# fabrizio-m/TyPLONK

Measured on AMD Instinct MI355X. Metric: msm_g1_adds_per_s, higher is better.
Workload: dtype u32; 1 GPU; 2^20-term BLS12-381 G1 MSM (KZG commit of a 2^20-row polynomial), SRS [s^i]G with s=2, 1048579 points; window_bits=20, windows=13, parallelism=single GPU, fixed_base_tables=c=20, 13 tables per rank

## Files before the change

### typlonk_amd/build.py

```python
from __future__ import annotations

import os
import shutil
import subprocess

ROOT = os.path.dirname(os.path.dirname(os.path.abspath(__file__)))
CSRC = os.path.join(ROOT, "typlonk_amd", "csrc")
LIB = os.path.join(ROOT, "typlonk_amd", "libtyplonk_hip.so")


def _stale(out: str, srcs: list[str]) -> bool:
    if not os.path.exists(out):
        return True
    t = os.path.getmtime(out)
    return any(os.path.getmtime(s) > t for s in srcs if os.path.exists(s))


def _run(cmd: list[str]) -> None:
    print("+", " ".join(cmd), flush=True)
    subprocess.run(cmd, check=True)


def hipcc_path() -> str:
    p = shutil.which("hipcc") or "/opt/rocm/bin/hipcc"
    if not os.path.exists(p):
        raise RuntimeError("hipcc not found: the HIP library cannot be built (there is no CPU fallback)")
    return p


HIP_UNITS = ["ctx.hip", "ntt_host.hip", "msm_host.hip", "comm.hip", "prover.hip", "ntt_kernels.hip", "msm_sort.hip", "msm_accum.hip", "msm_reduce.hip", "srs_gen.hip", "quotient.hip", "plonk_ops.hip", "poly_eval.hip", "verify.hip", "prove_batch.hip", "point_codec.hip", "witness_check.hip", "perm_pairs.hip", "witness_solve.hip"]
UNIT_FLAGS: dict[str, list[str]] = {}


def build_hip(force: bool = False) -> str:
    from concurrent.futures import ThreadPoolExecutor

    hdrs = [os.path.join(CSRC, f) for f in os.listdir(CSRC) if f.endswith(".hpp")]
    hdrs.append(os.path.join(ROOT, "include", "typlonk.h"))
    objdir = os.path.join(CSRC, "_obj")
    os.makedirs(objdir, exist_ok=True)
    hipcc = hipcc_path()
    jobs, objs = [], []
    for u in HIP_UNITS:
        src = os.path.join(CSRC, u)
        obj = os.path.join(objdir, u.replace(".hip", ".o"))
        objs.append(obj)
        if force or _stale(obj, [src] + hdrs):
            jobs.append([hipcc, "--offload-arch=gfx950", "-O3", "-std=c++17", "-fPIC", *UNIT_FLAGS.get(u, []), "-c", src, "-o", obj])
    if jobs:
        with ThreadPoolExecutor(max_workers=min(6, len(jobs))) as ex:
            list(ex.map(_run, jobs))
    if jobs or not os.path.exists(LIB):
        _run([hipcc, "--offload-arch=gfx950", "-shared", "-fPIC", *objs, "-o", LIB])
    return LIB


def build_hip_variant(name: str, unit_flags: dict[str, list[str]]) -> str:
    from concurrent.futures import ThreadPoolExecutor

    out_dir = os.path.join(ROOT, "tools", "_ab", name)
    os.makedirs(out_dir, exist_ok=True)
    hipcc = hipcc_path()
    base_obj = os.path.join(CSRC, "_obj")
    jobs, objs = [], []
    for u in HIP_UNITS:
        if u in unit_flags:
            obj = os.path.join(out_dir, u.replace(".hip", ".o"))
            jobs.append([hipcc, "--offload-arch=gfx950", "-O3", "-std=c++17", "-fPIC", *UNIT_FLAGS.get(u, []), *unit_flags[u], "-c",
                         os.path.join(CSRC, u), "-o", obj])
        else:
            obj = os.path.join(base_obj, u.replace(".hip", ".o"))
        objs.append(obj)
    build_hip()
    with ThreadPoolExecutor(max_workers=min(6, max(1, len(jobs)))) as ex:
        list(ex.map(_run, jobs))
    lib = os.path.join(out_dir, "libtyplonk_hip.so")
    _run([hipcc, "--offload-arch=gfx950", "-shared", "-fPIC", *objs, "-o", lib])
    return lib


def build_hip_test_hooks(force: bool = False) -> str:
    out_dir = os.path.join(ROOT, "tests", "cpp", "hooks")
    os.makedirs(out_dir, exist_ok=True)
    lib = os.path.join(out_dir, "libtyplonk_hip.so")
    hipcc = hipcc_path()
    build_hip()
    hdrs = [os.path.join(CSRC, f) for f in os.listdir(CSRC) if f.endswith(".hpp")] + [os.path.join(ROOT, "include", "typlonk.h")]
    src = os.path.join(CSRC, "comm.hip")
    obj = os.path.join(out_dir, "comm.o")
    base_obj = os.path.join(CSRC, "_obj")
    objs = [obj if u == "comm.hip" else os.path.join(base_obj, u.replace(".hip", ".o")) for u in HIP_UNITS]
    if force or _stale(obj, [src] + hdrs + [LIB]):
        _run([hipcc, "--offload-arch=gfx950", "-O3", "-std=c++17", "-fPIC", "-DTYPLONK_TEST_HOOKS", "-c", src, "-o", obj])
    if force or _stale(lib, objs):
        _run([hipcc, "--offload-arch=gfx950", "-shared", "-fPIC", *objs, "-o", lib])
    return lib


def build_host_shim(force: bool = False) -> str:
    src = os.path.join(ROOT, "tests", "cpp", "ff_host_shim.cpp")
    out = os.path.join(ROOT, "tests", "cpp", "libff_host_shim.so")
    deps = [src, os.path.join(CSRC, "ff.hpp"), os.path.join(CSRC, "g1.hpp"), os.path.join(CSRC, "fq30.hpp"), os.path.join(CSRC, "g1_host64.hpp"),
            os.path.join(CSRC, "fr30.hpp"), os.path.join(CSRC, "fr_inv.hpp"), os.path.join(CSRC, "transcript.hpp"), os.path.join(CSRC, "lin_commit.hpp")]
    if force or _stale(out, deps):
        _run(["g++", "-O2", "-std=c++17", "-shared", "-fPIC", src, "-o", out])
    return out


def build_device_arith(force: bool = False) -> str:
    src = os.path.join(ROOT, "tests", "cpp", "device_arith.hip")
    out = os.path.join(ROOT, "tests", "cpp", "libdevice_arith.so")
    hdrs = [os.path.join(CSRC, f) for f in os.listdir(CSRC) if f.endswith(".hpp")]
    if force or _stale(out, [src] + hdrs):
        _run([hipcc_path(), "--offload-arch=gfx950", "-O3", "-std=c++17", "-fPIC", "-shared", src, "-o", out])
    return out


def build_device_reduce(force: bool = False) -> str:
    src = os.path.join(CSRC, "harness", "device_reduce.hip")
    out = os.path.join(ROOT, "tests", "cpp", "libdevice_reduce.so")
    deps = [os.path.join(CSRC, f) for f in os.listdir(CSRC) if f.endswith(".hpp")] + [os.path.join(CSRC, "msm_reduce.hip")]
    if force or _stale(out, [src] + deps):
        _run([hipcc_path(), "--offload-arch=gfx950", "-O3", "-std=c++17", "-fPIC", "-shared", src, "-o", out])
    return out


def build_fq30_pair_host(force: bool = False) -> str:
    src = os.path.join(ROOT, "tests", "cpp", "fq30_pair_host.cpp")
    out = os.path.join(ROOT, "tests", "cpp", "libfq30_pair_host.so")
    deps = [src, os.path.join(ROOT, "tests", "cpp", "fq30_pair_harness.hpp"), os.path.join(CSRC, "ff.hpp"), os.path.join(CSRC, "fq30.hpp")]
    if force or _stale(out, deps):
        _run(["g++", "-O2", "-std=c++17", "-shared", "-fPIC", src, "-o", out])
    return out


def build_sigma_cell_host(force: bool = False) -> str:
    src = os.path.join(ROOT, "tests", "cpp", "sigma_cell_host.cpp")
    out = os.path.join(ROOT, "tests", "cpp", "libsigma_cell_host.so")
    deps = [src, os.path.join(CSRC, "ff.hpp"), os.path.join(CSRC, "sigma_cell.hpp")]
    if force or _stale(out, deps):
        _run(["g++", "-O2", "-std=c++17", "-shared", "-fPIC", src, "-o", out])
    return out


# ... 1 lines not shown
    src = os.path.join(ROOT, "tests", "cpp", "perm_pairs_host.cpp")
    out = os.path.join(ROOT, "tests", "cpp", "perm_pairs_host")
    deps = [src, os.path.join(CSRC, "ff.hpp"), os.path.join(CSRC, "perm_pairs.hpp")]
    if force or _stale(out, deps):
        _run(["g++", "-O2", "-std=c++17", "-pthread", src, "-o", out])
    return out


def build_msm_plan_host(force: bool = False) -> str:
    src = os.path.join(ROOT, "tests", "cpp", "msm_plan_host.cpp")
    out = os.path.join(ROOT, "tests", "cpp", "msm_plan_host")
    deps = [src, os.path.join(CSRC, "ff.hpp"), os.path.join(CSRC, "msm_plan.hpp")]
    if force or _stale(out, deps):
        _run(["g++", "-O2", "-std=c++17", src, "-o", out])
    return out


def build_ntt_plan_host(force: bool = False) -> str:
    src = os.path.join(ROOT, "tests", "cpp", "ntt_plan_host.cpp")
    out = os.path.join(ROOT, "tests", "cpp", "ntt_plan_host")
    deps = [src, os.path.join(CSRC, "ff.hpp"), os.path.join(CSRC, "fr30.hpp"), os.path.join(CSRC, "ntt_args.hpp"), os.path.join(CSRC, "ntt_plan.hpp")]
    if force or _stale(out, deps):
        _run(["g++", "-O2", "-std=c++17", src, "-o", out])
    return out


def build_prove_plan_host(force: bool = False, sanitize: bool = False) -> str:
    src = os.path.join(ROOT, "tests", "cpp", "prove_plan_host.cpp")
    out = os.path.join(ROOT, "tests", "cpp", "prove_plan_host_san" if sanitize else "prove_plan_host")
    deps = [src] + [os.path.join(CSRC, h) for h in ("ff.hpp", "fr30.hpp", "ntt_args.hpp", "ntt_plan.hpp", "prove_plan.hpp")]
    if force or _stale(out, deps):
        extra = ["-O1", "-g", "-fsanitize=address,undefined", "-fno-sanitize-recover=all"] if sanitize else ["-O2"]
        _run(["g++", *extra, "-std=c++17", src, "-o", out])
    return out


def build_solve_plan_host(force: bool = False, sanitize: bool = False) -> str:
    src = os.path.join(ROOT, "tests", "cpp", "solve_plan_host.cpp")
    out = os.path.join(ROOT, "tests", "cpp", "solve_plan_host_san" if sanitize else "solve_plan_host")
    deps = [src, os.path.join(CSRC, "solve_plan.hpp")]
    if force or _stale(out, deps):
        extra = ["-O1", "-g", "-fsanitize=address,undefined", "-fno-sanitize-recover=all"] if sanitize else ["-O2"]
        _run(["g++", *extra, "-std=c++17", src, "-o", out])
    return out


def build_madd_acc_host(force: bool = False, sanitize: bool = False) -> str:
    src = os.path.join(ROOT, "tests", "cpp", "madd_acc_host.cpp")
    out = os.path.join(ROOT, "tests", "cpp", "madd_acc_host_san" if sanitize else "madd_acc_host")
    deps = [src, os.path.join(CSRC, "ff.hpp"), os.path.join(CSRC, "fq30.hpp"), os.path.join(CSRC, "g1.hpp")]
    if force or _stale(out, deps):
        extra = ["-O1", "-g", "-fsanitize=address,undefined", "-fno-sanitize-recover=all"] if sanitize else ["-O2"]
        _run(["g++", *extra, "-std=c++17", src, "-o", out])
    return out


def build_device_pair(force: bool = False) -> str:
    src = os.path.join(ROOT, "tests", "cpp", "device_pair.hip")
    out = os.path.join(ROOT, "tests", "cpp", "libdevice_pair.so")
    hdrs = [os.path.join(CSRC, f) for f in os.listdir(CSRC) if f.endswith(".hpp")]
    hdrs.append(os.path.join(ROOT, "tests", "cpp", "fq30_pair_harness.hpp"))
    if force or _stale(out, [src] + hdrs):
        _run([hipcc_path(), "--offload-arch=gfx950", "-O3", "-std=c++17", "-fPIC", "-shared", src, "-o", out])
    return out


def build_host_tests(force: bool = False) -> list[str]:
    outs = []
    hdr = [os.path.join(ROOT, "typlonk_amd", "host", "typlonk_host.hpp"), os.path.join(ROOT, "typlonk_amd", "host", "pairing_host.hpp"),
           os.path.join(ROOT, "tests", "cpp", "circuit_host.hpp"),
           os.path.join(CSRC, "ff.hpp"), os.path.join(CSRC, "fq30.hpp"), os.path.join(CSRC, "g1_host64.hpp"),
           os.path.join(CSRC, "transcript.hpp"), LIB]
    for name in ("test_poly_host", "test_kzg_host", "test_plonk_host", "test_pairing_host", "test_circuit_tables_host", "test_circuit_host",
                 "test_comm_host", "test_comm_ranks_host", "test_compact_ranks_host", "test_verify_host", "test_prove_batch_host", "test_compact_host",
                 "test_prove_batch_compact_host", "test_wire_host", "test_witness_check_host", "test_circuit_compile_host",
                 "test_circuit_pairs_host", "test_witness_solve_host"):
        src = os.path.join(ROOT, "tests", "cpp", name + ".cpp")
        out = os.path.join(ROOT, "tests", "cpp", name)
        if force or _stale(out, [src] + hdr):
            _run(["g++", "-O2", "-std=c++17", src, "-o", out, "-L", os.path.join(ROOT, "typlonk_amd"), "-ltyplonk_hip",
                  "-Wl,-rpath," + os.path.join(ROOT, "typlonk_amd"), "-Wl,-rpath,$ORIGIN/../../typlonk_amd"])
        outs.append(out)
    return outs


def build_fake_rccl(force: bool = False) -> str:
    src = os.path.join(ROOT, "tests", "cpp", "fake_rccl.cpp")
    out = os.path.join(ROOT, "tests", "cpp", "libfake_rccl.so")
    if force or _stale(out, [src]):
        _run([hipcc_path(), "-O2", "-std=c++17", "-shared", "-fPIC", "-x", "hip", "--offload-arch=gfx950", src, "-o", out, "-lrt"])
    return out


def build_all(force: bool = False) -> None:
    build_hip(force)
    build_hip_test_hooks(force)
    build_host_shim(force)
    build_device_arith(force)
    build_device_reduce(force)
    build_fq30_pair_host(force)
    build_sigma_cell_host(force)
    build_perm_pairs_host(force)
    if os.path.exists(os.path.join(ROOT, "tests", "cpp", "msm_plan_host.cpp")):
        build_msm_plan_host(force)
    if os.path.exists(os.path.join(ROOT, "tests", "cpp", "ntt_plan_host.cpp")):
        build_ntt_plan_host(force)
    if os.path.exists(os.path.join(ROOT, "tests", "cpp", "prove_plan_host.cpp")):
        build_prove_plan_host(force)
        build_prove_plan_host(force, sanitize=True)
    if os.path.exists(os.path.join(ROOT, "tests", "cpp", "madd_acc_host.cpp")):
        build_madd_acc_host(force)
        build_madd_acc_host(force, sanitize=True)
    if os.path.exists(os.path.join(ROOT, "tests", "cpp", "solve_plan_host.cpp")):
        build_solve_plan_host(force)
        build_solve_plan_host(force, sanitize=True)
    build_device_pair(force)
    build_host_tests(force)
    build_fake_rccl(force)


if __name__ == "__main__":
    import sys

    if len(sys.argv) >= 3 and sys.argv[1] == "variant":
        flags: dict[str, list[str]] = {}
        for spec in sys.argv[3:]:
            unit, _, fl = spec.partition(":")
            flags[unit] = [f for f in fl.split(",") if f]
        print(build_hip_variant(sys.argv[2], flags))
    else:
        build_all()
```

### typlonk_amd/csrc/launch.hpp

```cpp
#pragma once
#include <hip/hip_runtime.h>
#include <stdint.h>
#include "ff.hpp"
#include "msm_plan.hpp"
#include "ntt_args.hpp"

namespace ty {

constexpr int PT_WORDS = 32;
constexpr int MSM_HEAVY_GRID = 1024;

struct QuotientArgs {
    const Fr* wires[3];
    const Fr* z;
    const Fr* sel[5];
    const Fr* sigma[3];
    const Fr* pi;
    const Fr* l0;
    const Fr* w_lo;
    const Fr* bx_hi;
    Fr* out;
    uint64_t n4;
    uint32_t w_h;
    uint32_t k0_is_one;
// ... 15 lines not shown
    uint64_t n;
    uint32_t w_h;
    Fr beta, gamma;
    Fr kbeta[3];
};
void launch_gp_terms(const GrandProductArgs& a, hipStream_t s);
void launch_product_scan(const Fr* in, uint64_t n, int reverse, Fr* block_scratch, Fr* out, hipStream_t s);
void launch_fr_inv(const Fr* in, Fr* out, hipStream_t s);
void launch_gp_finish(const Fr* nprefix, const Fr* dsuffix, const Fr* inv_total , uint64_t n, Fr* z, hipStream_t s);

void launch_open(const Fr* c, uint64_t m, const Fr& z, Fr* q, Fr* blocks, Fr* y, hipStream_t s);
struct LincombArgs {
    const Fr* poly[12];
    Fr scalar[12];
    Fr constant;
    Fr* out;
    uint64_t n;
    uint32_t terms;
};
void launch_lincomb(const LincombArgs& a, hipStream_t s);
void launch_open_multi(const Fr* const* polys, Fr* const* quotients, Fr* const* ys, const uint8_t* zsel, uint32_t count,
                       uint64_t m, const Fr& z0, const Fr& z1, Fr* blocks, hipStream_t s);

bool ntt_big_tiles_available();
void launch_ntt_pass(const NttPassArgs& a, unsigned blocks, unsigned threads, size_t lds_bytes, hipStream_t s);
void launch_ntt_pass30(const NttPassArgs& a, unsigned blocks, unsigned threads, size_t lds_bytes, hipStream_t s);
void launch_ntt_full_table(const Fr* lo, const Fr* hi, uint32_t h, uint64_t S, uint64_t n, Fr* out, hipStream_t s);

void launch_convert_points(uint32_t* pts, const uint8_t* inf, uint64_t n, hipStream_t s);
void launch_msm_digits(const Fr* scalars, uint64_t m, uint32_t c, uint32_t W, uint32_t top_v, uint32_t* keys,
                       uint32_t* counts, hipStream_t s);
void launch_scan(const uint32_t* counts, uint64_t n, uint32_t* block_sums, uint32_t* offsets, uint32_t* cursor,
                 hipStream_t s);
struct MsmSortPtrs {
    uint32_t *blk_hist, *blk_base, *scan_scratch, *blk_cnt, *seg_start, *entries, *counts, *offsets, *sorted, *hist514, *heavy, *tasks,
        *order;
};
void launch_msm_segsort(const Fr* scalars, uint64_t m, const MsmShape& sh, const MsmSortPtrs& p, uint32_t cap, int staged_mode,
                        hipStream_t s);
size_t srs_tables_scratch_bytes(uint64_t len, uint32_t T);
void launch_srs_tables(uint32_t* pts, uint32_t* zbuf, uint64_t len, uint32_t c, uint32_t T, hipStream_t s);
void launch_bucket_order(const uint32_t* counts, const uint32_t* offsets, uint32_t n, uint32_t cap, uint32_t* hist514,
                         uint32_t* order, uint32_t* heavy, uint32_t* tasks, hipStream_t s);
void launch_msm_heavy(const uint32_t* points, const uint32_t* sorted, const uint32_t* hist516, uint32_t* heavy,
                      const uint32_t* tasks, uint32_t* partial, uint32_t* buckets, hipStream_t s);
void launch_msm_scatter(const uint32_t* keys, uint64_t m, uint64_t total, uint32_t* cursor, uint32_t* sorted,
                        hipStream_t s);
void launch_msm_accum(const uint32_t* points, const uint32_t* offsets, const uint32_t* sorted, const uint32_t* order,
                      uint32_t nbuckets, uint32_t cap, bool init, uint32_t lanes, uint32_t split, uint32_t* buckets,
                      hipStream_t s);

void launch_msm_rc_reduce(const uint32_t* buckets, const RcShape& sh, uint32_t* pb, uint32_t* pa, uint32_t* sums,
                          uint32_t* bitsum, uint32_t* out, hipStream_t s);
void launch_msm_rc2_reduce(const uint32_t* buckets, const RcShape& sh, uint32_t* prow, uint32_t* pcol, uint32_t* out,
                           hipStream_t s);
void launch_msm_rc_combine(const uint32_t* planes, const RcShape& sh, uint32_t* set_sums, hipStream_t s);
void launch_fq_inv_selftest(uint64_t seed, uint32_t threads, uint32_t per_thread, uint32_t* out, hipStream_t st);
size_t srs_comb_bytes();
void launch_srs_comb(uint32_t* comb, hipStream_t st);
void launch_srs_generate(const Fr& s, uint64_t start, uint64_t n, const uint32_t* comb, uint32_t* pts, hipStream_t st);

}
```

### typlonk_amd/csrc/msm_reduce.hip

```cpp
#include "launch.hpp"
#include "msm_common.hpp"

namespace ty {

__global__ __launch_bounds__(64) void msm_rc_partial_kernel(const uint32_t* __restrict__ buckets, RcShape sh,
                                                            uint32_t nrow, uint32_t nrow_pad, uint32_t ncol,
                                                            uint32_t* pb, uint32_t* pa) {
    const uint32_t t = blockIdx.x * 64 + threadIdx.x;
    if (t < nrow_pad) {
        if (t >= nrow) return;
        const uint64_t base = (uint64_t)t << sh.llc;
        G1Xyzz v = ld_xyzz(buckets, base);
        for (uint32_t l = 1; l < (1u << sh.llc); ++l) v = g1_add(v, ld_xyzz(buckets, base + l));
        st_xyzz(pb, t, v);
        return;
    }
    const uint32_t u = t - nrow_pad;
    if (u >= ncol) return;
    const uint32_t per_set = sh.c1 - sh.lhc;
    const uint32_t set = u >> per_set, rem = u & ((1u << per_set) - 1);
    const uint32_t lo = rem & ((1u << sh.cl) - 1), hchunk = rem >> sh.cl;
    const uint64_t first = ((uint64_t)set << sh.c1) + ((uint64_t)(hchunk << sh.lhc) << sh.cl) + lo;
    G1Xyzz v = ld_xyzz(buckets, first);
    for (uint32_t h = 1; h < (1u << sh.lhc); ++h) v = g1_add(v, ld_xyzz(buckets, first + ((uint64_t)h << sh.cl)));
    st_xyzz(pa, ((((uint64_t)set << sh.cl) + lo) << (sh.ch - sh.lhc)) + hchunk, v);
}

struct FoldSeg {
    const uint32_t* in;
    uint32_t* out;
    uint32_t threads, lseq, lanes;
};
__global__ __launch_bounds__(256) void msm_fold_seq_kernel(FoldSeg a, FoldSeg b, uint32_t waves_a, uint32_t waves) {
    const uint32_t wv = blockIdx.x * 4 + (threadIdx.x >> 6);
    if (wv >= waves) return;
    const bool first = wv < waves_a;
    const FoldSeg& g = first ? a : b;
    const uint32_t t = (wv - (first ? 0u : waves_a)) * 64 + (threadIdx.x & 63u);
    G1Xyzz v = G1Xyzz::inf();
    if (t < g.threads) {
        const uint64_t base = (uint64_t)t << g.lseq;
        v = ld_xyzz(g.in, base);
        for (uint32_t i = 1; i < (1u << g.lseq); ++i) v = g1_add(v, ld_xyzz(g.in, base + i));
    }
    v = butterfly_reduce(v, g.lanes);
    if (t < g.threads && (t & (g.lanes - 1)) == 0) st_xyzz(g.out, t / g.lanes, v);
}

__global__ __launch_bounds__(64) void msm_rc_bits_kernel(const uint32_t* __restrict__ sums, RcShape sh, uint32_t rw,
                                                         uint32_t cw, uint32_t* bitsum) {
    const uint32_t nbr_max = sh.ch + 1, nbc_max = sh.cl + 1;
    const uint32_t wps = nbr_max * rw + nbc_max * cw;
// ... 107 lines not shown
    v = G1Xyzz::inf();
    if (threadIdx.x < 2 * nwaves) {
        const uint32_t w = threadIdx.x >> 1;
#pragma unroll
        for (int i = 0; i < 13; ++i) {
            v.x.v[i] = xch[w][i];
            v.y.v[i] = xch[w][13 + i];
            v.zz.v[i] = xch[w][26 + i];
            v.zzz.v[i] = xch[w][39 + i];
        }
    }
#pragma unroll 1
    for (int mask = 2; mask < (int)(2 * nwaves); mask <<= 1) v = butterfly_add4(v, mask);
    if (threadIdx.x == 0) st_xyzz(out, blockIdx.x, v);
}

constexpr uint32_t RC2_LOG_WAVES = 10;
void launch_msm_rc2_reduce(const uint32_t* buckets, const RcShape& sh, uint32_t* prow, uint32_t* pcol, uint32_t* out,
                           hipStream_t s) {
    uint32_t lnb = sh.c1;
    for (uint32_t n = sh.nsets; n > 1; n >>= 1) ++lnb;
    const uint32_t want = lnb > 5 + RC2_LOG_WAVES ? lnb - 5 - RC2_LOG_WAVES : 0;
    const uint32_t sr = want < sh.cl - 6 ? want : sh.cl - 6, sc = want < sh.ch - 6 ? want : sh.ch - 6;
    const uint32_t nwave_row = sh.nsets << (sh.c1 - 6 - sr), nwave_col = sh.nsets << (sh.c1 - 6 - sc);
    hipLaunchKernelGGL(msm_rc2_sums_kernel, dim3((nwave_row + nwave_col + 3) / 4), dim3(256), 0, s, buckets, sh, sr, sc, nwave_row,
                       nwave_row + nwave_col, prow, pcol);
    const uint32_t lpr = sh.cl - 6 - sr, lpc = sh.ch - 6 - sc;
    uint32_t np = 1u << ((sh.ch + lpr) > (sh.cl + lpc) ? (sh.ch + lpr) : (sh.cl + lpc));
    if (sh.top_v == 0 && np > 64) np >>= 1;
    const uint32_t threads = np < 64 ? 64u : (np > (uint32_t)RC2_THREADS ? (uint32_t)RC2_THREADS : np);
    hipLaunchKernelGGL(msm_rc2_planes_kernel, dim3(sh.nsets * 2 * RC_NB), dim3(threads), 0, s, prow, pcol, sh, lpr, lpc, out);
}

__global__ __launch_bounds__(64) void msm_rc_combine_kernel(const uint32_t* __restrict__ planes, RcShape sh,
                                                            uint32_t* set_sums) {
    const uint32_t set = blockIdx.x, kind = threadIdx.x / RC_NB, b = threadIdx.x % RC_NB;
    uint32_t nbr, nbc, shift;
    rc_bits(sh, set, &nbr, &nbc, &shift);
    const bool valid = kind < 2 && b < (kind ? nbc : nbr);
    G1Xyzz v = G1Xyzz::inf();
    if (valid) v = ld_xyzz(planes, (uint64_t)(set * 2 + kind) * RC_NB + b);
    const uint32_t e = valid ? b + (kind ? 0u : shift) : 0u;
    const uint32_t emax = max(nbr ? nbr - 1 + shift : 0u, nbc ? nbc - 1 : 0u);
    for (uint32_t i = 0; i < emax; ++i)
        if (i < e) v = g1_dbl(v);
    for (uint32_t mask = 1; mask < 2 * RC_NB; mask <<= 1) v = butterfly_add(v, (int)mask);
    if (threadIdx.x == 0) st_xyzz(set_sums, set, v);
}

void launch_msm_rc_combine(const uint32_t* planes, const RcShape& sh, uint32_t* set_sums, hipStream_t s) {
    hipLaunchKernelGGL(msm_rc_combine_kernel, dim3(sh.nsets), dim3(64), 0, s, planes, sh, set_sums);
}

void launch_msm_rc_reduce(const uint32_t* buckets, const RcShape& sh, uint32_t* pb, uint32_t* pa, uint32_t* sums,
                          uint32_t* bitsum, uint32_t* out, hipStream_t s) {
    const uint32_t nrow = sh.nsets << (sh.c1 - sh.llc), ncol = sh.nsets << (sh.c1 - sh.lhc);
    const uint32_t nrow_pad = (nrow + 63) & ~63u;
    hipLaunchKernelGGL(msm_rc_partial_kernel, dim3((nrow_pad + ncol + 63) / 64), dim3(64), 0, s, buckets, sh, nrow, nrow_pad,
                       ncol, pb, pa);
    auto seg = [](const uint32_t* in, uint32_t* out, uint32_t n_in, uint32_t lcnt) {
        FoldSeg g;
        g.in = in;
        g.out = out;
        g.lseq = lcnt < 1 ? lcnt : 1;
        g.lanes = 1u << (lcnt - g.lseq);
        g.threads = n_in >> g.lseq;
        return g;
    };
    uint32_t* rsum = sums;
    uint32_t* csum = sums + ((uint64_t)sh.nsets << sh.ch) * 48;
    const FoldSeg a = seg(pb, rsum, nrow, sh.cl - sh.llc), b = seg(pa, csum, ncol, sh.ch - sh.lhc);
    const uint32_t ba = (a.threads + 63) / 64, bb = (b.threads + 63) / 64;
    hipLaunchKernelGGL(msm_fold_seq_kernel, dim3((ba + bb + 3) / 4), dim3(256), 0, s, a, b, ba, ba + bb);
    if (sh.ch >= 6 && sh.cl >= 6) {
        uint32_t np = 1u << (sh.ch > sh.cl ? sh.ch : sh.cl);
        if (sh.top_v == 0 && np > 64) np >>= 1;
        const uint32_t threads = np < 64 ? 64u : (np > (uint32_t)RC2_THREADS ? (uint32_t)RC2_THREADS : np);
        hipLaunchKernelGGL(msm_rc2_planes_kernel, dim3(sh.nsets * 2 * RC_NB), dim3(threads), 0, s, rsum, csum, sh, 0u, 0u, out);
        return;
    }
    const uint32_t rw = ((1u << sh.ch) + 63) / 64, cw = ((1u << sh.cl) + 63) / 64;
    const uint32_t wps = (sh.ch + 1) * rw + (sh.cl + 1) * cw;
    hipLaunchKernelGGL(msm_rc_bits_kernel, dim3(sh.nsets * wps), dim3(64), 0, s, sums, sh, rw, cw, bitsum);
    hipLaunchKernelGGL(msm_rc_final_kernel, dim3(sh.nsets * 2 * RC_NB), dim3(64), 0, s, bitsum, sh, rw, cw, out);
}

}
```

Baseline: 6.741 billion G1-adds/s.

## Reduce MSM bit planes with limb-parallel row point additions

Adds a limb-parallel field representation where 16 lanes hold one Fq element and four lane groups cooperate on an XYZZ point addition, using DPP broadcasts and Montgomery multiply across lanes. The row/column bit-plane reduction now runs a two-stage shared-memory tree of these cooperative additions instead of the previous per-thread rc2 planes kernel. The goal is to spread the final bucket-reduction stage over more lanes and raise occupancy, at the cost of cross-lane traffic and lazy-reduction carry handling. Build-script shortcuts and test harnesses are also added.

```diff
diff --git a/typlonk_amd/build.py b/typlonk_amd/build.py
--- a/typlonk_amd/build.py
+++ b/typlonk_amd/build.py
@@ -38,6 +38,8 @@
     hdrs = [os.path.join(CSRC, f) for f in os.listdir(CSRC) if f.endswith(".hpp")]
     hdrs.append(os.path.join(ROOT, "include", "typlonk.h"))
     objdir = os.path.join(CSRC, "_obj")
+    if not force and not _stale(LIB, [os.path.join(CSRC, u) for u in HIP_UNITS] + hdrs):
+        return LIB
     os.makedirs(objdir, exist_ok=True)
     hipcc = hipcc_path()
     jobs, objs = [], []
@@ -90,6 +92,10 @@
     obj = os.path.join(out_dir, "comm.o")
     base_obj = os.path.join(CSRC, "_obj")
     objs = [obj if u == "comm.hip" else os.path.join(base_obj, u.replace(".hip", ".o")) for u in HIP_UNITS]
+    if not force and not _stale(lib, [src] + hdrs + [LIB]):
+        return lib
+    if not all(os.path.exists(o) for o in objs if o != obj):
+        build_hip(force=True)
     if force or _stale(obj, [src] + hdrs + [LIB]):
         _run([hipcc, "--offload-arch=gfx950", "-O3", "-std=c++17", "-fPIC", "-DTYPLONK_TEST_HOOKS", "-c", src, "-o", obj])
     if force or _stale(lib, objs):
@@ -197,6 +203,25 @@
     if force or _stale(out, deps):
         extra = ["-O1", "-g", "-fsanitize=address,undefined", "-fno-sanitize-recover=all"] if sanitize else ["-O2"]
         _run(["g++", *extra, "-std=c++17", src, "-o", out])
+    return out
+
+
+def build_fq30_rows_host(force: bool = False, sanitize: bool = False) -> str:
+    src = os.path.join(ROOT, "tests", "cpp", "fq30_rows_host.cpp")
+    out = os.path.join(ROOT, "tests", "cpp", "fq30_rows_host_san" if sanitize else "fq30_rows_host")
+    deps = [src] + [os.path.join(CSRC, h) for h in ("ff.hpp", "fq30.hpp", "g1.hpp", "fq30_rows.hpp")]
+    if force or _stale(out, deps):
+        extra = ["-O1", "-g", "-fsanitize=address,undefined", "-fno-sanitize-recover=all"] if sanitize else ["-O2"]
+        _run(["g++", *extra, "-std=c++17", src, "-o", out])
+    return out
+
+
+def build_device_reduce_rows(force: bool = False) -> str:
+    src = os.path.join(CSRC, "harness", "device_reduce_rows.hip")
+    out = os.path.join(ROOT, "tests", "cpp", "libdevice_reduce_rows.so")
+    deps = [os.path.join(CSRC, f) for f in os.listdir(CSRC) if f.endswith(".hpp")] + [os.path.join(CSRC, "msm_reduce.hip")]
+    if force or _stale(out, [src] + deps):
+        _run([hipcc_path(), "--offload-arch=gfx950", "-O3", "-std=c++17", "-fPIC", "-shared", src, "-o", out])
     return out
 
 
@@ -259,6 +284,10 @@
     if os.path.exists(os.path.join(ROOT, "tests", "cpp", "solve_plan_host.cpp")):
         build_solve_plan_host(force)
         build_solve_plan_host(force, sanitize=True)
+    if os.path.exists(os.path.join(ROOT, "tests", "cpp", "fq30_rows_host.cpp")):
+        build_fq30_rows_host(force)
+        build_fq30_rows_host(force, sanitize=True)
+    build_device_reduce_rows(force)
     build_device_pair(force)
     build_host_tests(force)
     build_fake_rccl(force)
diff --git a/typlonk_amd/csrc/fq30_rows.hpp b/typlonk_amd/csrc/fq30_rows.hpp
--- /dev/null
+++ b/typlonk_amd/csrc/fq30_rows.hpp
@@ -0,0 +1,402 @@
+#pragma once
+#include "g1.hpp"
+
+namespace ty {
+
+constexpr uint32_t FQR_LOOSE = (1u << 30) + 3u;
+
+#if defined(__HIPCC__)
+struct RowsDev {
+    using U32 = uint32_t;
+    using U64 = uint64_t;
+    using Mask = bool;
+    static __device__ __forceinline__ U32 limb() { return threadIdx.x & 15u; }
+    static __device__ __forceinline__ U32 role() { return (threadIdx.x >> 4) & 3u; }
+    static __device__ __forceinline__ U32 splat(uint32_t v) { return v; }
+    static __device__ __forceinline__ U32 bcast(U32 x, int k) {
+#define FQR_BC(K) case K: return (U32)__builtin_amdgcn_mov_dpp((int)x, 0x150 + K, 0xf, 0xf, false)
+        switch (k) {
+            FQR_BC(0); FQR_BC(1); FQR_BC(2); FQR_BC(3); FQR_BC(4); FQR_BC(5); FQR_BC(6); FQR_BC(7);
+            FQR_BC(8); FQR_BC(9); FQR_BC(10); FQR_BC(11); FQR_BC(12); FQR_BC(13); FQR_BC(14);
+            default: FQR_BC(15);
+        }
+#undef FQR_BC
+    }
+    static __device__ __forceinline__ U32 up1(U32 x) { return (U32)__builtin_amdgcn_update_dpp(0, (int)x, 0x111, 0xf, 0xf, true); }
+    static __device__ __forceinline__ U32 down1(U32 x) { return (U32)__builtin_amdgcn_update_dpp(0, (int)x, 0x101, 0xf, 0xf, true); }
+    static __device__ __forceinline__ U32 xrow(U32 x, int m) { return (U32)__shfl_xor((int)x, m << 4); }
+    static __device__ __forceinline__ U64 zero64() { return 0; }
+    static __device__ __forceinline__ U64 mad(U32 a, U32 b, U64 acc) { return acc + (uint64_t)a * b; }
+    static __device__ __forceinline__ U32 lo(U64 a) { return (U32)a; }
+    static __device__ __forceinline__ U64 shr30_add(U64 a, U32 x) { return (a >> 30) + x; }
+    static __device__ __forceinline__ U32 sel(Mask c, U32 a, U32 b) { return c ? a : b; }
+    static __device__ __forceinline__ bool any(Mask m) { return __any((int)m) != 0; }
+    static __device__ __forceinline__ Mask row_all(Mask m) {
+        const uint64_t b = __ballot((int)m);
+        return ((b >> (threadIdx.x & 48u)) & 0xffffu) == 0xffffu;
+    }
+    static __device__ __forceinline__ U32 load2(const uint32_t* p0, const uint32_t* p1, Mask second, U32 idx) {
+        return (second ? p1 : p0)[idx];
+    }
+    static __device__ __forceinline__ void store(uint32_t* p, U32 idx, U32 v, Mask m) {
+        if (m) p[idx] = v;
+    }
+    static __device__ __forceinline__ U32 lane_table(const uint32_t (&t)[16]) {
+        U32 r = 0;
+        const U32 l = limb();
+#pragma unroll
+        for (int i = 0; i < 13; ++i) r = l == (U32)i ? t[i] : r;
+        return r;
+    }
+};
+#endif
+#if !defined(__HIP_DEVICE_COMPILE__)
+template <class T>
+struct HV {
+    T l[64];
+};
+#define FQR_HV_BIN(OP)                                                        \
+    template <class T>                                                        \
+    inline HV<T> operator OP(const HV<T>& a, const HV<T>& b) {                \
+        HV<T> r;                                                              \
+        for (int i = 0; i < 64; ++i) r.l[i] = (T)(a.l[i] OP b.l[i]);          \
+        return r;                                                             \
+    }                                                                         \
+    template <class T>                                                        \
+    inline HV<T> operator OP(const HV<T>& a, uint32_t b) {                    \
+        HV<T> r;                                                              \
+        for (int i = 0; i < 64; ++i) r.l[i] = (T)(a.l[i] OP (T)b);            \
+        return r;                                                             \
+    }
+FQR_HV_BIN(+)
+FQR_HV_BIN(-)
+FQR_HV_BIN(*)
+FQR_HV_BIN(&)
+FQR_HV_BIN(|)
+#undef FQR_HV_BIN
+inline HV<uint32_t> operator>>(const HV<uint32_t>& a, const HV<uint32_t>& n) {
+    HV<uint32_t> r;
+    for (int i = 0; i < 64; ++i) r.l[i] = a.l[i] >> (n.l[i] & 31u);
+    return r;
+}
+inline HV<uint32_t> operator<<(const HV<uint32_t>& a, const HV<uint32_t>& n) {
+    HV<uint32_t> r;
+    for (int i = 0; i < 64; ++i) r.l[i] = a.l[i] << (n.l[i] & 31u);
+    return r;
+}
+inline HV<uint32_t> operator>>(const HV<uint32_t>& a, int n) {
+    HV<uint32_t> r;
+    for (int i = 0; i < 64; ++i) r.l[i] = a.l[i] >> n;
+    return r;
+}
+#define FQR_HV_CMP(OP)                                                        \
+    inline HV<bool> operator OP(const HV<uint32_t>& a, const HV<uint32_t>& b) { \
+        HV<bool> r;                                                           \
+        for (int i = 0; i < 64; ++i) r.l[i] = a.l[i] OP b.l[i];               \
+        return r;                                                             \
+    }                                                                         \
+    inline HV<bool> operator OP(const HV<uint32_t>& a, uint32_t b) {          \
+        HV<bool> r;                                                           \
+        for (int i = 0; i < 64; ++i) r.l[i] = a.l[i] OP b;                    \
+        return r;                                                             \
+    }
+FQR_HV_CMP(==)
+FQR_HV_CMP(!=)
+FQR_HV_CMP(<)
+#undef FQR_HV_CMP
+inline HV<bool> operator&&(const HV<bool>& a, const HV<bool>& b) {
+    HV<bool> r;
+    for (int i = 0; i < 64; ++i) r.l[i] = a.l[i] && b.l[i];
+    return r;
+}
+inline HV<bool> operator||(const HV<bool>& a, const HV<bool>& b) {
+    HV<bool> r;
+    for (int i = 0; i < 64; ++i) r.l[i] = a.l[i] || b.l[i];
+    return r;
+}
+inline HV<bool> operator!(const HV<bool>& a) {
+    HV<bool> r;
+    for (int i = 0; i < 64; ++i) r.l[i] = !a.l[i];
+    return r;
+}
+
+struct RowsHost {
+    using U32 = HV<uint32_t>;
+    using U64 = HV<uint64_t>;
+    using Mask = HV<bool>;
+    static U32 limb() {
+        U32 r;
+        for (int i = 0; i < 64; ++i) r.l[i] = (uint32_t)i & 15u;
+        return r;
+    }
+    static U32 role() {
+        U32 r;
+        for (int i = 0; i < 64; ++i) r.l[i] = (uint32_t)i >> 4;
+        return r;
+    }
+    static U32 splat(uint32_t v) {
+        U32 r;
+        for (int i = 0; i < 64; ++i) r.l[i] = v;
+        return r;
+    }
+    static U32 bcast(const U32& x, int k) {
+        U32 r;
+        for (int i = 0; i < 64; ++i) r.l[i] = x.l[(i & 48) | k];
+        return r;
+    }
+    static U32 up1(const U32& x) {
+        U32 r;
+        for (int i = 0; i < 64; ++i) r.l[i] = (i & 15) ? x.l[i - 1] : 0u;
+        return r;
+    }
+    static U32 down1(const U32& x) {
+        U32 r;
+        for (int i = 0; i < 64; ++i) r.l[i] = (i & 15) != 15 ? x.l[i + 1] : 0u;
+        return r;
+    }
+    static U32 xrow(const U32& x, int m) {
+        U32 r;
+        for (int i = 0; i < 64; ++i) r.l[i] = x.l[i ^ (m << 4)];
+        return r;
+    }
+    static U64 zero64() {
+        U64 r;
+        for (int i = 0; i < 64; ++i) r.l[i] = 0;
+        return r;
+    }
+    static U64 mad(const U32& a, const U32& b, const U64& acc) {
+        U64 r;
+        for (int i = 0; i < 64; ++i) {
+            const uint64_t t = (uint64_t)a.l[i] * b.l[i];
+            r.l[i] = acc.l[i] + t;
+            if (r.l[i] < t) overflow() = true;
+        }
+        return r;
+    }
+    static bool& overflow() {
+        static bool f = false;
+        return f;
+    }
+    static U32 lo(const U64& a) {
+        U32 r;
+        for (int i = 0; i < 64; ++i) r.l[i] = (uint32_t)a.l[i];
+        return r;
+    }
+    static U64 shr30_add(const U64& a, const U32& x) {
+        U64 r;
+        for (int i = 0; i < 64; ++i) r.l[i] = (a.l[i] >> 30) + x.l[i];
+        return r;
+    }
+    static U32 sel(const Mask& c, const U32& a, const U32& b) {
+        U32 r;
+        for (int i = 0; i < 64; ++i) r.l[i] = c.l[i] ? a.l[i] : b.l[i];
+        return r;
+    }
+    static bool any(const Mask& m) {
+        for (int i = 0; i < 64; ++i)
+            if (m.l[i]) return true;
+        return false;
+    }
+    static Mask row_all(const Mask& m) {
+        Mask r;
+        for (int row = 0; row < 4; ++row) {
+            bool a = true;
+            for (int i = 0; i < 16; ++i) a = a && m.l[row * 16 + i];
+            for (int i = 0; i < 16; ++i) r.l[row * 16 + i] = a;
+        }
+        return r;
+    }
+    static U32 load2(const uint32_t* p0, const uint32_t* p1, const Mask& second, const U32& idx) {
+        U32 r;
+        for (int i = 0; i < 64; ++i) r.l[i] = (second.l[i] ? p1 : p0)[idx.l[i]];
+        return r;
+    }
+    static void store(uint32_t* p, const U32& idx, const U32& v, const Mask& m) {
+        for (int i = 0; i < 64; ++i)
+            if (m.l[i]) p[idx.l[i]] = v.l[i];
+    }
+    static U32 lane_table(const uint32_t (&t)[16]) {
+        U32 r;
+        for (int i = 0; i < 64; ++i) r.l[i] = t[i & 15];
+        return r;
+    }
+};
+#endif
+
+template <class W>
+TY_HD typename W::U32 fqr_p() {
+    const uint32_t t[16] = {fq30_kp(1, 0), fq30_kp(1, 1), fq30_kp(1, 2), fq30_kp(1, 3), fq30_kp(1, 4), fq30_kp(1, 5), fq30_kp(1, 6),
+                            fq30_kp(1, 7), fq30_kp(1, 8), fq30_kp(1, 9), fq30_kp(1, 10), fq30_kp(1, 11), fq30_kp(1, 12), 0, 0, 0};
+    return W::lane_table(t);
+}
+TY_HD constexpr uint32_t fqr_kp_lent(int k, int j) {
+    return j == 0 ? fq30_kp(k, 0) + (1u << 30) : j < 12 ? fq30_kp(k, j) + (1u << 30) - 1u : fq30_kp(k, 12) - 1u;
+}
+TY_HD constexpr bool fqr_kp_digits_ok() {
+    for (int k = 1; k <= 8; ++k) {
+        for (int j = 0; j < 12; ++j)
+            if (fq30_kp(k, j) < 4u) return false;
+        if (fq30_kp(k, 12) < 1u) return false;
+    }
+    return true;
+}
+static_assert(fqr_kp_digits_ok(), "a lent digit of K p could go negative against a loose limb");
+template <class W, int K>
+TY_HD typename W::U32 fqr_kp_lent_lanes() {
+    const uint32_t t[16] = {fqr_kp_lent(K, 0), fqr_kp_lent(K, 1), fqr_kp_lent(K, 2), fqr_kp_lent(K, 3), fqr_kp_lent(K, 4),
+                            fqr_kp_lent(K, 5), fqr_kp_lent(K, 6), fqr_kp_lent(K, 7), fqr_kp_lent(K, 8), fqr_kp_lent(K, 9),
+                            fqr_kp_lent(K, 10), fqr_kp_lent(K, 11), fqr_kp_lent(K, 12), 0, 0, 0};
+    return W::lane_table(t);
+}
+
+template <class W>
+TY_HD typename W::U32 fqr_norm(const typename W::U32& s) {
+    return (s & FQ30_MASK) + W::up1(s >> 30);
+}
+template <class W>
+TY_HD typename W::U32 fqr_full_norm(typename W::U32 s) {
+    for (int it = 0; it < 14; ++it) {
+        const typename W::U32 c = s >> 30;
+        if (!W::any(c != 0u)) break;
+        s = (s & FQ30_MASK) + W::up1(c);
+    }
+    return s;
+}
+
+template <class W>
+TY_HD typename W::U32 fqr_mul(const typename W::U32& a, const typename W::U32& b) {
+    const typename W::U32 p = fqr_p<W>();
+    typename W::U64 acc = W::zero64();
+#pragma unroll
+    for (int i = 0; i < 13; ++i) {
+        acc = W::mad(W::bcast(a, i), b, acc);
+        const typename W::U32 m = (W::lo(acc) * FQ30_NINV) & FQ30_MASK;
+        acc = W::mad(W::bcast(m, 0), p, acc);
+        acc = W::shr30_add(acc, W::down1(W::lo(acc)) & FQ30_MASK);
+    }
+    return fqr_norm<W>(W::lo(acc));
+}
+
+template <class W>
+TY_HD typename W::U32 fqr_add_lazy(const typename W::U32& a, const typename W::U32& b) {
+    return fqr_norm<W>(a + b);
+}
+template <class W, int K>
+TY_HD typename W::U32 fqr_mulk_lazy(const typename W::U32& a) {
+    return fqr_norm<W>(a * (uint32_t)K);
+}
+template <class W, int K>
+TY_HD typename W::U32 fqr_sub_lazy(const typename W::U32& a, const typename W::U32& b) {
+    return fqr_norm<W>(a + fqr_kp_lent_lanes<W, K>() - b);
+}
+template <class W, int K>
+TY_HD typename W::U32 fqr_sub2_lazy(const typename W::U32& a, const typename W::U32& b, const typename W::U32& c) {
+    return fqr_sub_lazy<W, K>(a, fqr_add_lazy<W>(b, c));
+}
+template <class W>
+TY_HD typename W::U32 fqr_select(const typename W::Mask& c, const typename W::U32& a, const typename W::U32& b) {
+    return W::sel(c, a, b);
+}
+template <class W>
+TY_HD typename W::Mask fqr_is_zero_mod(const typename W::U32& a) {
+    const typename W::U32 d = fqr_full_norm<W>(a);
+    return W::row_all(d == 0u) || W::row_all(d == fqr_p<W>());
+}
+template <class W>
+TY_HD typename W::Mask fqr_maybe_zero_mod(const typename W::U32& a) {
+    const typename W::U32 low = a & FQ30_MASK;
+    return (W::limb() == 0u) && (low == 0u || low == fq30_kp(1, 0));
+}
+
+TY_HD uint32_t fqr_limb_of_words(const uint32_t* w, uint32_t i) {
+    if (i > 12u) return 0u;
+    const uint32_t cur = i < 12u ? w[i] : 0u;
+    if (i == 0u) return cur & FQ30_MASK;
+    return ((w[i - 1] >> (32u - 2u * i)) | (cur << (2u * i))) & FQ30_MASK;
+}
+template <class W>
+TY_HD typename W::U32 fqr_load(const uint32_t* w) {
+    const typename W::U32 i = W::limb();
+    const typename W::Mask has = i < 12u;
+    const typename W::U32 cur = W::sel(has, W::load2(w, w, has, W::sel(has, i, W::splat(0))), W::splat(0));
+    const typename W::U32 below = W::up1(cur);
+    const typename W::U32 hi = W::sel(i == 0u, W::splat(0), below >> ((W::splat(32) - i * 2u) & 31u));
+    return W::sel(i < 13u, (hi | (cur << (i * 2u))) & FQ30_MASK, W::splat(0));
+}
+template <class W>
+TY_HD void fqr_store_rows(uint32_t* w, const typename W::U32& a) {
+    const typename W::U32 d = fqr_full_norm<W>(a);
+    const typename W::U32 j = W::limb();
+    const typename W::U32 word = (d >> (j * 2u)) | (W::down1(d) << (W::splat(30) - j * 2u));
+    W::store(w, W::role() * 12u + j, word, j < 12u);
+}
+
+constexpr uint32_t FQR_POINT_WORDS = 64;
+
+TY_HD Fq30 fqr_to_fq30(const uint32_t* l) {
+    Fq30 r;
+    uint32_t c = 0;
+    for (int i = 0; i < 13; ++i) {
+        const uint32_t s = l[i] + c;
+        r.v[i] = s & FQ30_MASK;
+        c = s >> 30;
+    }
+    return r;
+}
+TY_HD G1Xyzz fqr_to_xyzz(const uint32_t* pt) {
+    G1Xyzz r;
+    r.x = fqr_to_fq30(pt);
+    r.y = fqr_to_fq30(pt + 16);
+    r.zz = fqr_to_fq30(pt + 32);
+    r.zzz = fqr_to_fq30(pt + 48);
+    return r;
+}
+
+template <class W>
+TY_HD bool g1_add_rows(const uint32_t* A, const uint32_t* B, uint32_t* out) {
+    using U32 = typename W::U32;
+    using Mask = typename W::Mask;
+    const U32 li = W::limb(), role = W::role();
+    const Mask odd = (role & 1u) != 0u, bside = (role & 2u) != 0u;
+    const U32 zoff = W::sel(odd, W::splat(48), W::splat(32)) + li;
+    const U32 own = W::load2(A, B, bside, W::sel(odd, W::splat(16), W::splat(0)) + li);
+    const U32 oz = W::load2(A, B, !bside, zoff);
+    const U32 mz = W::load2(A, B, bside, zoff);
+    const U32 m1 = fqr_mul<W>(own, oz);
+    const U32 x1 = W::xrow(m1, 2);
+    const U32 d = fqr_sub_lazy<W, 2>(W::sel(bside, m1, x1), W::sel(bside, x1, m1));
+    const U32 m2 = fqr_mul<W>(W::sel(bside, d, mz), W::sel(bside, d, oz));
+    const Mask maybe = (!odd && fqr_maybe_zero_mod<W>(mz)) || (bside && !odd && fqr_maybe_zero_mod<W>(m2));
+    if (W::any(maybe)) {
+        const G1Xyzz s = g1_add(fqr_to_xyzz(A), fqr_to_xyzz(B));
+        const uint32_t tx[16] = {s.x.v[0], s.x.v[1], s.x.v[2], s.x.v[3], s.x.v[4], s.x.v[5], s.x.v[6], s.x.v[7], s.x.v[8], s.x.v[9],
+                                 s.x.v[10], s.x.v[11], s.x.v[12], 0, 0, 0};
+        const uint32_t ty[16] = {s.y.v[0], s.y.v[1], s.y.v[2], s.y.v[3], s.y.v[4], s.y.v[5], s.y.v[6], s.y.v[7], s.y.v[8], s.y.v[9],
+                                 s.y.v[10], s.y.v[11], s.y.v[12], 0, 0, 0};
+        const uint32_t tz[16] = {s.zz.v[0], s.zz.v[1], s.zz.v[2], s.zz.v[3], s.zz.v[4], s.zz.v[5], s.zz.v[6], s.zz.v[7], s.zz.v[8],
+                                 s.zz.v[9], s.zz.v[10], s.zz.v[11], s.zz.v[12], 0, 0, 0};
+        const uint32_t tw[16] = {s.zzz.v[0], s.zzz.v[1], s.zzz.v[2], s.zzz.v[3], s.zzz.v[4], s.zzz.v[5], s.zzz.v[6], s.zzz.v[7],
+                                 s.zzz.v[8], s.zzz.v[9], s.zzz.v[10], s.zzz.v[11], s.zzz.v[12], 0, 0, 0};
+        const U32 v = W::sel(bside, W::sel(odd, W::lane_table(tw), W::lane_table(tz)), W::sel(odd, W::lane_table(ty), W::lane_table(tx)));
+        W::store(out, role * 16u + li, v, li < 16u);
+        return true;
+    }
+    const U32 x2 = W::xrow(m2, 2);
+    const U32 m3 = fqr_mul<W>(W::sel(bside, d, m1), W::sel(bside, m2, x2));
+    const U32 qa = W::xrow(m3, 1);
+    const U32 qb = W::xrow(m3, 3);
+    const U32 qc = W::xrow(m2, 3);
+    const U32 x3 = fqr_sub2_lazy<W, 4>(x2, qb, fqr_mulk_lazy<W, 2>(qa));
+    const U32 t = fqr_sub_lazy<W, 6>(qa, x3);
+    const U32 opa = W::sel(bside, W::sel(odd, x1, qc), W::sel(odd, d, m2));
+    const U32 opb = W::sel(bside, W::sel(odd, qa, m3), W::sel(odd, t, x2));
+    const U32 m4 = fqr_mul<W>(opa, opb);
+    const U32 y3 = fqr_sub_lazy<W, 2>(m4, W::xrow(m4, 2));
+    W::store(out, li, x3, role == 1u);
+    W::store(out, li + 16u, y3, role == 1u);
+    W::store(out, li + 32u, m4, role == 0u);
+    W::store(out, li + 48u, m4, role == 2u);
+    return false;
+}
+
+}
diff --git a/typlonk_amd/csrc/harness/device_reduce_rows.hip b/typlonk_amd/csrc/harness/device_reduce_rows.hip
--- /dev/null
+++ b/typlonk_amd/csrc/harness/device_reduce_rows.hip
@@ -0,0 +1,112 @@
+#include "../msm_reduce.hip"
+
+#include <algorithm>
+
+using namespace ty;
+
+namespace {
+
+struct Bufs {
+    void* p[8] = {};
+    int used = 0;
+    hipError_t err = hipSuccess;
+    uint32_t* zeros(uint64_t points) {
+        void* d = nullptr;
+        const size_t bytes = (size_t)std::max<uint64_t>(points, 1) * 192;
+        if (err == hipSuccess) err = hipMalloc(&d, bytes);
+        if (err == hipSuccess) p[used++] = d;
+        if (err == hipSuccess) err = hipMemset(d, 0, bytes);
+        return static_cast<uint32_t*>(d);
+    }
+    ~Bufs() {
+        for (int i = 0; i < used; ++i) (void)hipFree(p[i]);
+    }
+};
+
+bool shape_ok(const RcShape& sh) {
+    if (sh.nsets < 1 || sh.nsets > 32 || sh.c1 != sh.cl + sh.ch || sh.c1 > 19) return false;
+    if (sh.cl < 6 || sh.ch < 6 || sh.cl > 12 || sh.ch > 12 || sh.lhc > sh.ch || sh.llc > sh.cl) return false;
+    if (sh.cl - sh.llc > 7 || sh.ch - sh.lhc > 7) return false;
+    for (uint32_t set = 0; set < sh.nsets; ++set) {
+        uint32_t nbr, nbc, shift;
+        rc_bits(sh, set, &nbr, &nbc, &shift);
+        if (nbr > RC_NB || nbc > RC_NB) return false;
+    }
+    return true;
+}
+
+__global__ __launch_bounds__(256) void add_pairs_kernel(const uint32_t* __restrict__ a, const uint32_t* __restrict__ b, uint32_t npairs,
+                                                        uint32_t* rows_out, uint32_t* lane_out, uint32_t* slow) {
+    __shared__ uint32_t buf[4][3][FQR_POINT_WORDS];
+    const uint32_t wave = threadIdx.x >> 6, lane = threadIdx.x & 63u, w = blockIdx.x * 4 + wave;
+    if (w >= npairs) return;
+    const uint32_t c = lane >> 4, i = lane & 15u;
+    buf[wave][0][lane] = fqr_limb_of_words(a + (uint64_t)w * 48 + c * 12, i);
+    buf[wave][1][lane] = fqr_limb_of_words(b + (uint64_t)w * 48 + c * 12, i);
+    __builtin_amdgcn_fence(__ATOMIC_RELEASE, "wavefront");
+    __builtin_amdgcn_wave_barrier();
+    __builtin_amdgcn_fence(__ATOMIC_ACQUIRE, "wavefront");
+    const bool s = g1_add_rows<RowsDev>(buf[wave][0], buf[wave][1], buf[wave][2]);
+    __builtin_amdgcn_fence(__ATOMIC_RELEASE, "wavefront");
+    __builtin_amdgcn_wave_barrier();
+    __builtin_amdgcn_fence(__ATOMIC_ACQUIRE, "wavefront");
+    fqr_store_rows<RowsDev>(rows_out + (uint64_t)w * 48, buf[wave][2][lane]);
+    if (lane == 0) {
+        slow[w] = s ? 1u : 0u;
+        st_xyzz(lane_out, w, g1_add(ld_xyzz(a, w), ld_xyzz(b, w)));
+    }
+}
+
+}
+
+extern "C" int drr_add_pairs(const uint32_t* a, const uint32_t* b, uint32_t npairs, uint32_t* rows_out, uint32_t* lane_out,
+                             uint32_t* slow) {
+    if (npairs < 1 || npairs > 4096) return (int)hipErrorInvalidValue;
+    Bufs m;
+    uint32_t* d_a = m.zeros(npairs);
+    uint32_t* d_b = m.zeros(npairs);
+    uint32_t* d_r = m.zeros(npairs);
+    uint32_t* d_l = m.zeros(npairs);
+    uint32_t* d_s = m.zeros((npairs + 47) / 48);
+    if (m.err == hipSuccess) m.err = hipMemcpy(d_a, a, (size_t)npairs * 192, hipMemcpyHostToDevice);
+    if (m.err == hipSuccess) m.err = hipMemcpy(d_b, b, (size_t)npairs * 192, hipMemcpyHostToDevice);
+    if (m.err == hipSuccess) {
+        hipLaunchKernelGGL(add_pairs_kernel, dim3((npairs + 3) / 4), dim3(256), 0, 0, d_a, d_b, npairs, d_r, d_l, d_s);
+        m.err = hipGetLastError();
+    }
+    if (m.err == hipSuccess) m.err = hipDeviceSynchronize();
+    if (m.err == hipSuccess) m.err = hipMemcpy(rows_out, d_r, (size_t)npairs * 192, hipMemcpyDeviceToHost);
+    if (m.err == hipSuccess) m.err = hipMemcpy(lane_out, d_l, (size_t)npairs * 192, hipMemcpyDeviceToHost);
+    if (m.err == hipSuccess) m.err = hipMemcpy(slow, d_s, (size_t)npairs * 4, hipMemcpyDeviceToHost);
+    return (int)m.err;
+}
+
+extern "C" int drr_reduce(int form, const uint32_t* shape, const uint32_t* buckets, uint32_t* planes) {
+    RcShape sh;
+    sh.nsets = shape[0];
+    sh.c1 = shape[1];
+    sh.ch = shape[2];
+    sh.cl = shape[3];
+    sh.lhc = shape[4];
+    sh.llc = shape[5];
+    sh.top_v = shape[6];
+    if ((form != 0 && form != 1) || !shape_ok(sh) || !msm_rows_ok(sh)) return (int)hipErrorInvalidValue;
+    const uint64_t nb = (uint64_t)sh.nsets << sh.c1;
+    const uint64_t nrow = (uint64_t)sh.nsets << (sh.c1 - sh.llc), ncol = (uint64_t)sh.nsets << (sh.c1 - sh.lhc);
+    const uint64_t nplanes = (uint64_t)sh.nsets * 2 * RC_NB;
+    Bufs m;
+    uint32_t* d_buckets = m.zeros(nb);
+    uint32_t* part_b = m.zeros(nrow);
+    uint32_t* part_a = m.zeros(ncol);
+    uint32_t* sums = m.zeros(((uint64_t)sh.nsets << sh.ch) + ((uint64_t)sh.nsets << sh.cl));
+    uint32_t* bitsum = m.zeros(nplanes * 64);
+    uint32_t* d_planes = m.zeros(nplanes);
+    if (m.err == hipSuccess) m.err = hipMemcpy(d_buckets, buckets, (size_t)nb * 192, hipMemcpyHostToDevice);
+    if (m.err == hipSuccess) {
+        launch_msm_rc_reduce_form(d_buckets, sh, part_b, part_a, sums, bitsum, d_planes, form == 0, 0);
+        m.err = hipGetLastError();
+    }
+    if (m.err == hipSuccess) m.err = hipDeviceSynchronize();
+    if (m.err == hipSuccess) m.err = hipMemcpy(planes, d_planes, (size_t)nplanes * 192, hipMemcpyDeviceToHost);
+    return (int)m.err;
+}
diff --git a/typlonk_amd/csrc/launch.hpp b/typlonk_amd/csrc/launch.hpp
--- a/typlonk_amd/csrc/launch.hpp
+++ b/typlonk_amd/csrc/launch.hpp
@@ -91,6 +91,8 @@
 
 void launch_msm_rc_reduce(const uint32_t* buckets, const RcShape& sh, uint32_t* pb, uint32_t* pa, uint32_t* sums,
                           uint32_t* bitsum, uint32_t* out, hipStream_t s);
+void launch_msm_rc_reduce_form(const uint32_t* buckets, const RcShape& sh, uint32_t* pb, uint32_t* pa, uint32_t* sums,
+                               uint32_t* bitsum, uint32_t* out, bool rows, hipStream_t s);
 void launch_msm_rc2_reduce(const uint32_t* buckets, const RcShape& sh, uint32_t* prow, uint32_t* pcol, uint32_t* out,
                            hipStream_t s);
 void launch_msm_rc_combine(const uint32_t* planes, const RcShape& sh, uint32_t* set_sums, hipStream_t s);
diff --git a/typlonk_amd/csrc/msm_reduce.hip b/typlonk_amd/csrc/msm_reduce.hip
--- a/typlonk_amd/csrc/msm_reduce.hip
+++ b/typlonk_amd/csrc/msm_reduce.hip
@@ -1,3 +1,4 @@
+#include "fq30_rows.hpp"
 #include "launch.hpp"
 #include "msm_common.hpp"
 
@@ -211,8 +212,89 @@
     hipLaunchKernelGGL(msm_rc_combine_kernel, dim3(sh.nsets), dim3(64), 0, s, planes, sh, set_sums);
 }
 
-void launch_msm_rc_reduce(const uint32_t* buckets, const RcShape& sh, uint32_t* pb, uint32_t* pa, uint32_t* sums,
-                          uint32_t* bitsum, uint32_t* out, hipStream_t s) {
+constexpr uint32_t ROWS_MAX_ITEMS = 64;
+constexpr int ROWS_THREADS0 = 256, ROWS_THREADS1 = 512;
+
+struct RowsPlane {
+    uint32_t set, kind, bit, v, litems, nsel, ng;
+    bool top, live;
+};
+__device__ __forceinline__ RowsPlane rows_plane(const RcShape& sh, uint32_t plane, uint32_t ln1) {
+    RowsPlane p;
+    p.bit = plane % RC_NB;
+    p.kind = (plane / RC_NB) & 1u;
+    p.set = plane / (2 * RC_NB);
+    uint32_t nbr, nbc, shift;
+    rc_bits(sh, p.set, &nbr, &nbc, &shift);
+    p.live = p.bit < (p.kind ? nbc : nbr);
+    p.v = rc_set_v(sh, p.set);
+    p.litems = p.kind ? sh.cl : sh.ch;
+    p.top = p.v == 0 && p.kind && p.bit == sh.cl;
+    p.nsel = p.v == 0 ? (p.top ? 1u : 1u << (p.litems - 1)) : 1u << p.litems;
+    p.ng = (p.nsel + (1u << ln1) - 1) >> ln1;
+    return p;
+}
+__device__ __forceinline__ const uint32_t* rows_item(const RcShape& sh, const RowsPlane& p, const uint32_t* rsum,
+                                                     const uint32_t* csum, uint32_t idx) {
+    const uint32_t* src = p.kind ? csum : rsum;
+    const uint64_t sbase = (uint64_t)p.set << p.litems;
+    if (p.v == 0) {
+        const uint32_t w = p.top ? (1u << sh.cl) : (((idx >> p.bit) << (p.bit + 1)) | (1u << p.bit) | (idx & ((1u << p.bit) - 1)));
+        return src + (sbase + (w - p.kind)) * 48;
+    }
+    return ((rc_weight(sh, p.set, p.kind, idx) >> p.bit) & 1u) ? src + (sbase + idx) * 48 : nullptr;
+}
+__device__ __forceinline__ uint32_t rows_inf_limb(uint32_t c, uint32_t i) {
+    uint32_t r = 0;
+#pragma unroll
+    for (int j = 0; j < 13; ++j) r = (c < 2 && i == (uint32_t)j) ? fq30_one_limb(j) : r;
+    return r;
+}
+
+template <int STAGE>
+__global__ __launch_bounds__(STAGE ? ROWS_THREADS1 : ROWS_THREADS0) void msm_rows_planes_kernel(
+    const uint32_t* __restrict__ rsum, const uint32_t* __restrict__ csum, RcShape sh, uint32_t ln1, uint32_t G, uint32_t* part,
+    uint32_t* out) {
+    __shared__ uint32_t buf0[ROWS_MAX_ITEMS * FQR_POINT_WORDS];
+    __shared__ uint32_t buf1[ROWS_MAX_ITEMS / 2 * FQR_POINT_WORDS];
+    const uint32_t plane = STAGE ? blockIdx.x : blockIdx.x / G, g = STAGE ? 0u : blockIdx.x % G;
+    const RowsPlane p = rows_plane(sh, plane, ln1);
+    if (!p.live || g >= p.ng) return;
+    const uint32_t first = g << ln1;
+    const uint32_t valid = STAGE ? p.ng : min(1u << ln1, p.nsel - first);
+    uint32_t n = 1;
+    while (n < valid) n <<= 1;
+    for (uint32_t e = threadIdx.x; e < n * FQR_POINT_WORDS; e += blockDim.x) {
+        const uint32_t k = e >> 6, c = (e >> 4) & 3u, i = e & 15u;
+        const uint32_t* src = nullptr;
+        if (k < valid) src = STAGE ? part + ((uint64_t)plane * 64 + k) * 48 : rows_item(sh, p, rsum, csum, first + k);
+        buf0[e] = src ? fqr_limb_of_words(src + c * 12, i) : rows_inf_limb(c, i);
+    }
+    const uint32_t wave = threadIdx.x >> 6, nwaves = blockDim.x >> 6;
+    uint32_t* cur = buf0;
+    uint32_t* nxt = buf1;
+#pragma unroll 1
+    for (uint32_t cnt = n; cnt > 1; cnt >>= 1) {
+        __syncthreads();
+#pragma unroll 1
+        for (uint32_t a = wave; a < cnt / 2; a += nwaves)
+            g1_add_rows<RowsDev>(cur + (2 * a) * FQR_POINT_WORDS, cur + (2 * a + 1) * FQR_POINT_WORDS, nxt + a * FQR_POINT_WORDS);
+        uint32_t* t = cur;
+        cur = nxt;
+        nxt = t;
+    }
+    __syncthreads();
+    uint32_t* dst = STAGE ? out + (uint64_t)plane * 48 : part + ((uint64_t)plane * 64 + g) * 48;
+    if (wave == 0) fqr_store_rows<RowsDev>(dst, cur[threadIdx.x]);
+}
+
+static bool msm_rows_ok(const RcShape& sh) {
+    const uint32_t lmax = sh.ch > sh.cl ? sh.ch : sh.cl;
+    return sh.ch >= 6 && sh.cl >= 6 && lmax - (sh.top_v == 0 ? 1u : 0u) <= 12;
+}
+
+void launch_msm_rc_reduce_form(const uint32_t* buckets, const RcShape& sh, uint32_t* pb, uint32_t* pa, uint32_t* sums,
+                               uint32_t* bitsum, uint32_t* out, bool rows, hipStream_t s) {
     const uint32_t nrow = sh.nsets << (sh.c1 - sh.llc), ncol = sh.nsets << (sh.c1 - sh.lhc);
     const uint32_t nrow_pad = (nrow + 63) & ~63u;
     hipLaunchKernelGGL(msm_rc_partial_kernel, dim3((nrow_pad + ncol + 63) / 64), dim3(64), 0, s, buckets, sh, nrow, nrow_pad,
@@ -231,6 +313,15 @@
     const FoldSeg a = seg(pb, rsum, nrow, sh.cl - sh.llc), b = seg(pa, csum, ncol, sh.ch - sh.lhc);
     const uint32_t ba = (a.threads + 63) / 64, bb = (b.threads + 63) / 64;
     hipLaunchKernelGGL(msm_fold_seq_kernel, dim3((ba + bb + 3) / 4), dim3(256), 0, s, a, b, ba, ba + bb);
+    if (rows && msm_rows_ok(sh)) {
+        const uint32_t lmax = (sh.ch > sh.cl ? sh.ch : sh.cl) - (sh.top_v == 0 ? 1u : 0u);
+        const uint32_t ln1 = lmax > 10 ? lmax - 6 : 4;
+        const uint32_t G = lmax > ln1 ? 1u << (lmax - ln1) : 1u;
+        const uint32_t nplanes = sh.nsets * 2 * RC_NB;
+        hipLaunchKernelGGL(msm_rows_planes_kernel<0>, dim3(nplanes * G), dim3(ROWS_THREADS0), 0, s, rsum, csum, sh, ln1, G, bitsum, out);
+        hipLaunchKernelGGL(msm_rows_planes_kernel<1>, dim3(nplanes), dim3(ROWS_THREADS1), 0, s, rsum, csum, sh, ln1, G, bitsum, out);
+        return;
+    }
     if (sh.ch >= 6 && sh.cl >= 6) {
         uint32_t np = 1u << (sh.ch > sh.cl ? sh.ch : sh.cl);
         if (sh.top_v == 0 && np > 64) np >>= 1;
@@ -244,4 +335,9 @@
     hipLaunchKernelGGL(msm_rc_final_kernel, dim3(sh.nsets * 2 * RC_NB), dim3(64), 0, s, bitsum, sh, rw, cw, out);
 }
 
-}
+void launch_msm_rc_reduce(const uint32_t* buckets, const RcShape& sh, uint32_t* pb, uint32_t* pa, uint32_t* sums,
+                          uint32_t* bitsum, uint32_t* out, hipStream_t s) {
+    launch_msm_rc_reduce_form(buckets, sh, pb, pa, sums, bitsum, out, true, s);
+}
+
+}
```

Measured after the change: 6.858 billion G1-adds/s (median of 6 runs). 1.7% higher.
